# NethermindEth/stark-rings

Measured on AMD Instinct MI355X. Metric: ring-muls/sec (Goldilocks, deg 2^16, batch 2^14), higher is better.
Workload: dtype u64; 1 GPU; goldilocks_d65536_b16384; ring=goldilocks, degree=65536, batch_per_gpu=16384, global_batch=16384, layout=ark-ff Montgomery u64 limbs, in place (a *= b), b read-only, variant=mul, parallelism=batch-sharded x1, twiddle broadcast only

## Files before the change

stark_rings_amd/csrc/ntt_goldilocks.hpp:

```cpp
#pragma once
#include <utility>

#include "fields.hpp"

namespace sr {
namespace gl {

using G = Goldilocks;
typedef uint64_t u64;
typedef uint32_t u32;

constexpr int kW16Exp = 156;

__device__ __forceinline__ u64 ld_stream(const u64 *p) { return __builtin_nontemporal_load(p); }
__device__ __forceinline__ void st_stream(u64 *p, u64 v) { __builtin_nontemporal_store(v, p); }
__device__ __forceinline__ u64 ld_scratch(const u64 *p) { return *p; }
__device__ __forceinline__ void st_scratch(u64 *p, u64 v) { *p = v; }
__device__ __forceinline__ void st_result(u64 *p, u64 v) {
    repcheck::leaves_library(v);
    st_stream(p, v);
}
__device__ __forceinline__ void st_slots(u64 *p, u64 v) {
    repcheck::leaves_library(v);
    *p = v;
// ... 247 lines not shown
template <int E>
SR_HD u64 mul_pow2_signed(u64 x) {
    if constexpr (E == 0) return x;
    else if constexpr (E < 96) return mul_pow2<E>(x);
    else if constexpr (E == 96) return G::neg(x);
    else return G::neg(mul_pow2<E - 96>(x));
}
constexpr int twist_exp(int q) { return (39 << (q + 1)) % 192; }
template <int Q, bool INVERSE, int... Js>
SR_HD void twist_rows(u64 *x, std::integer_sequence<int, Js...>) {
    ((x[Js] = mul_pow2_signed<INVERSE ? (192 - (twist_exp(Q) * (Js & ((16 >> Q) - 1))) % 192) % 192
                                      : (twist_exp(Q) * (Js & ((16 >> Q) - 1))) % 192>(x[Js])),
     ...);
}

struct Tables {
    const u64 *tw, *itw;
    const u64 *twist_f;
    const u64 *twist_i_plain, *twist_i_mul;
    const u64 *w1f, *w1i, *w1i_mul;
    const u64 *w2f, *w2i;
    const u64 *wcf, *wci;
};

template <int M, int DIR, bool TWIST>
__global__ __launch_bounds__(256) void strided_kernel(u64 *data, const u64 *src, int k, int s_lo, const u64 *tw, const u64 *twist) {
    constexpr int R = 1 << M;
    const int ls = k - s_lo - M;
    const size_t S = (size_t)1 << ls;
    const unsigned chunks = (unsigned)(S >> 8);
    const unsigned ci = blockIdx.x % chunks;
    const unsigned rest = blockIdx.x / chunks;
    const unsigned h = rest & ((1u << s_lo) - 1u);
    const size_t poly = rest >> s_lo;
    const unsigned i = ci * 256u + threadIdx.x;
    const size_t off = (poly << k) + ((size_t)h << (k - s_lo)) + i;
    u64 *base = data + off;
    const u64 *sbase = src + off;

    u64 x[R];
#pragma unroll
    for (int j = 0; j < R; j++) x[j] = sbase[(size_t)j << ls];

    if (DIR == 0) {
#pragma unroll
        for (int t = 0; t < M; t++) {
            const int half = 1 << (M - 1 - t);
#pragma unroll
            for (int j = 0; j < R; j++) {
                if (j & half) continue;
                const u64 w = tw[(1u << (s_lo + t)) + (h << t) + (unsigned)(j >> (M - t))];
                const u64 u = x[j], v = G::mul(x[j + half], w);
                x[j] = G::add(u, v);
                x[j + half] = G::sub(u, v);
            }
        }
        if (TWIST) {
#pragma unroll
            for (int j = 0; j < R; j++) x[j] = G::mul(x[j], twist[((size_t)((h << M) + j) << 12) + i]);
        }
    } else {
        if (TWIST) {
#pragma unroll
            for (int j = 0; j < R; j++) x[j] = G::mul(x[j], twist[((size_t)((h << M) + j) << 12) + i]);
        }
#pragma unroll
        for (int t = M - 1; t >= 0; t--) {
            const int half = 1 << (M - 1 - t);
#pragma unroll
            for (int j = 0; j < R; j++) {
                if (j & half) continue;
                const u64 w = tw[(1u << (s_lo + t)) + (h << t) + (unsigned)(j >> (M - t))];
                const u64 u = x[j], v = x[j + half];
                x[j] = G::add(u, v);
                x[j + half] = G::mul(G::sub(u, v), w);
            }
        }
    }
#pragma unroll
    for (int j = 0; j < R; j++) base[(size_t)j << ls] = x[j];
}

__device__ __forceinline__ int pad(int pos);

template <int DIR, bool TWIST>
__global__ __launch_bounds__(256, 4) void strided256_kernel(u64 *data, const u64 *src, int k, int s_lo, const u64 *tw, const u64 *twist) {
    __shared__ u64 lds[kLdsElems];
    const int t = threadIdx.x;
    const int ls = k - s_lo - 8;
    const unsigned chunks = 1u << (ls - 4);
    const unsigned ci = blockIdx.x & (chunks - 1u);
    const unsigned rest = blockIdx.x >> (ls - 4);
    const unsigned h = rest & ((1u << s_lo) - 1u);
    const size_t poly = rest >> s_lo;
    const int col = t & 15, rg = t >> 4;
    const unsigned i = ci * 16u + (unsigned)col;
    const size_t off = (poly << k) + ((size_t)h << (k - s_lo)) + i;
    u64 *base = data + off;
    const u64 *sbase = src + off;
    const int base2 = rg * 256 + col;
    u64 x[16];

    if (DIR == 0) {
#pragma unroll
        for (int jj = 0; jj < 16; jj++) x[jj] = sbase[(size_t)(rg + 16 * jj) << ls];
#pragma unroll
        for (int u = 0; u < 4; u++) {
            const int half = 8 >> u;
#pragma unroll
            for (int jj = 0; jj < 16; jj++) {
                if (jj & half) continue;
                const u64 w = tw[(1u << (s_lo + u)) + (h << u) + (unsigned)(jj >> (4 - u))];
                const u64 a = x[jj], v = G::mul(x[jj + half], w);
                x[jj] = G::add(a, v);
                x[jj + half] = G::sub(a, v);
            }
        }
#pragma unroll
        for (int jj = 0; jj < 16; jj++) lds[pad(jj * 256 + t)] = x[jj];
        __syncthreads();
#pragma unroll
        for (int jj = 0; jj < 16; jj++) x[jj] = lds[pad(base2 + jj * 16)];
#pragma unroll
        for (int u = 0; u < 4; u++) {
            const int half = 8 >> u;
#pragma unroll
            for (int jj = 0; jj < 16; jj++) {
                if (jj & half) continue;
                const u64 w = tw[(1u << (s_lo + 4 + u)) + (h << (4 + u)) + ((unsigned)rg << u) + (unsigned)(jj >> (4 - u))];
                const u64 a = x[jj], v = G::mul(x[jj + half], w);
                x[jj] = G::add(a, v);
                x[jj + half] = G::sub(a, v);
            }
        }
#pragma unroll
        for (int jj = 0; jj < 16; jj++) {
            u64 v = x[jj];
            if (TWIST) v = G::mul(v, twist[((size_t)((h << 8) + (unsigned)(16 * rg + jj)) << 12) + i]);
            base[(size_t)(16 * rg + jj) << ls] = v;
        }
    } else {
#pragma unroll
        for (int jj = 0; jj < 16; jj++) {
            u64 v = sbase[(size_t)(16 * rg + jj) << ls];
            if (TWIST) v = G::mul(v, twist[((size_t)((h << 8) + (unsigned)(16 * rg + jj)) << 12) + i]);
            x[jj] = v;
        }
#pragma unroll
        for (int u = 3; u >= 0; u--) {
            const int half = 8 >> u;
#pragma unroll
            for (int jj = 0; jj < 16; jj++) {
                if (jj & half) continue;
                const u64 w = tw[(1u << (s_lo + 4 + u)) + (h << (4 + u)) + ((unsigned)rg << u) + (unsigned)(jj >> (4 - u))];
                const u64 a = x[jj], b = x[jj + half];
                x[jj] = G::add(a, b);
                x[jj + half] = G::mul(G::sub(a, b), w);
            }
        }
#pragma unroll
        for (int jj = 0; jj < 16; jj++) lds[pad(base2 + jj * 16)] = x[jj];
        __syncthreads();
#pragma unroll
        for (int jj = 0; jj < 16; jj++) x[jj] = lds[pad(jj * 256 + t)];
#pragma unroll
        for (int u = 3; u >= 0; u--) {
            const int half = 8 >> u;
#pragma unroll
            for (int jj = 0; jj < 16; jj++) {
                if (jj & half) continue;
                const u64 w = tw[(1u << (s_lo + u)) + (h << u) + (unsigned)(jj >> (4 - u))];
                const u64 a = x[jj], b = x[jj + half];
                x[jj] = G::add(a, b);
                x[jj + half] = G::mul(G::sub(a, b), w);
            }
        }
#pragma unroll
        for (int jj = 0; jj < 16; jj++) base[(size_t)(rg + 16 * jj) << ls] = x[jj];
    }
}

__device__ __forceinline__ int pad(int pos) { return pos + (pos >> 4); }

constexpr int brv5(int i) { return ((i & 1) << 4) | ((i & 2) << 2) | (i & 4) | ((i & 8) >> 2) | ((i & 16) >> 4); }
constexpr int cols_tw_exp(int i) { return (39 * brv5(i)) % 192; }
template <int U, bool INV>
struct ColsStageOf {
    template <int I>
    struct Bf {
        static constexpr int half = 8 >> U;
        static constexpr int lo = (I / half) * 2 * half + I % half, hi = lo + half;
        static constexpr int e = cols_tw_exp((1 << U) + (lo >> (4 - U)));
        static constexpr int E = INV ? (192 - e) % 192 : e;
    };
};
template <int U, int P = kPhased>
SR_HD void cols_stage_fwd(u64 *x) {
    stage_in_groups<ColsStageOf<U, false>::template Bf, true, 8, P, true>(x);
}
template <int U, int P = kPhased>
SR_HD void cols_stage_inv(u64 *x) {
    stage_in_groups<ColsStageOf<U, true>::template Bf, false, 8, P>(x);
}

template <int LC>
struct ColsTile {
    static constexpr int C = 1 << LC;
    static constexpr int kLanes = 16 * C;
    static constexpr int kElems = LC == 4 ? kLdsElems : 256 * C;
    static __device__ __forceinline__ int idx(int leg, int col) {
        const int pos = leg * C + col;
        return LC == 4 ? pos + (pos >> 4) : pos;
    }
};
template <int DIR, int LC>
__device__ __forceinline__ void cols256_tile(const unsigned tile, u64 *data, const u64 *src, int k, const u64 *__restrict__ wc,
                                             const u64 *__restrict__ twist, u64 *lds) {
    using CT = ColsTile<LC>;
    constexpr int C = CT::C;
    const int t = threadIdx.x;
    const int ls = k - 8;
    const unsigned ci = tile & ((1u << (ls - LC)) - 1u);
    const size_t poly = tile >> (ls - LC);
    const int col = t & (C - 1), rg = t >> LC;
    const unsigned i = ci * (unsigned)C + (unsigned)col;
    char *pb = reinterpret_cast<char *>(data + (poly << k));
    const char *ps = reinterpret_cast<const char *>(src + (poly << k));
    const char *tb = reinterpret_cast<const char *>(twist);
    const unsigned leg = 8u << ls;
    const unsigned offA = (((unsigned)rg << ls) + i) * 8u;
    const unsigned offB = (((unsigned)rg << (ls + 4)) + i) * 8u;
    u64 x[16];

    if (DIR == 0) {
#pragma unroll
        for (int jj = 0; jj < 16; jj++) x[jj] = ld_stream(reinterpret_cast<const u64 *>(ps + (offA + (unsigned)jj * 16u * leg)));
        cols_stage_fwd<0>(x);
        cols_stage_fwd<1>(x);
        cols_stage_fwd<2>(x);
        cols_stage_fwd<3>(x);
#pragma unroll
        for (int h = 0; h < 16; h++) x[h] = G::mul(x[h], wc[h * 16 + rg]);
#pragma unroll
        for (int h = 0; h < 16; h++) lds[CT::idx(16 * h + rg, col)] = x[h];
        __syncthreads();
        u64 tw[16];
#pragma unroll
        for (int sg = 0; sg < 16; sg++) tw[sg] = *reinterpret_cast<const u64 *>(tb + (offB + (unsigned)sg * leg));
#pragma unroll
        for (int j = 0; j < 16; j++) x[j] = lds[CT::idx(16 * rg + j, col)];
        dft16_fwd_hot(x);
#pragma unroll
        for (int sg = 0; sg < 16; sg++)
            st_scratch(reinterpret_cast<u64 *>(pb + (offB + (unsigned)sg * leg)), G::mul(x[sg], tw[sg]));
    } else {
        u64 tw[16];
#pragma unroll
        for (int sg = 0; sg < 16; sg++) {
            x[sg] = ld_scratch(reinterpret_cast<const u64 *>(ps + (offB + (unsigned)sg * leg)));
            tw[sg] = *reinterpret_cast<const u64 *>(tb + (offB + (unsigned)sg * leg));
        }
#pragma unroll
        for (int sg = 0; sg < 16; sg++) x[sg] = G::mul(x[sg], tw[sg]);
        dft16_inv_hot(x);
#pragma unroll
        for (int j = 0; j < 16; j++) lds[CT::idx(16 * rg + j, col)] = x[j];
        __syncthreads();
#pragma unroll
        for (int h = 0; h < 16; h++) x[h] = lds[CT::idx(16 * h + rg, col)];
#pragma unroll
        for (int h = 0; h < 16; h++) x[h] = G::mul(x[h], wc[h * 16 + rg]);
        cols_stage_inv<3>(x);
        cols_stage_inv<2>(x);
        cols_stage_inv<1>(x);
        cols_stage_inv<0>(x);
#pragma unroll
        for (int jj = 0; jj < 16; jj++) st_result(reinterpret_cast<u64 *>(pb + (offA + (unsigned)jj * 16u * leg)), x[jj]);
    }
}

constexpr int kColsXcdGroup = 4;
template <int DIR, int LC>
__global__ __launch_bounds__(16 << LC, 4) void cols256_kernel(u64 *data, const u64 *src, int k, const u64 *__restrict__ wc,
                                                              const u64 *__restrict__ twist, unsigned grouped) {
    __shared__ u64 lds[ColsTile<LC>::kElems];
    __shared__ u64 wl[256];
    if (threadIdx.x < 256) wl[threadIdx.x] = wc[threadIdx.x];
    __syncthreads();
    cols256_tile<DIR, LC>(xcd_tile(blockIdx.x, kColsXcdGroup, grouped), data, src, k, wl, twist, lds);
}
template <int LC>
__global__ __launch_bounds__(16 << LC, 4) void cols256_pair_kernel(u64 *data_a, const u64 *src_a, u64 *data_b, const u64 *src_b, int k,
                                                                   const u64 *__restrict__ wc, const u64 *__restrict__ twist,
                                                                   unsigned grouped, unsigned tiles) {
    __shared__ u64 lds[ColsTile<LC>::kElems];
    __shared__ u64 wl[256];
    if (threadIdx.x < 256) wl[threadIdx.x] = wc[threadIdx.x];
    __syncthreads();
    const unsigned v = xcd_tile(blockIdx.x, kColsXcdGroup, grouped);
    const bool second = v >= tiles;
    cols256_tile<0, LC>(second ? v - tiles : v, second ? data_b : data_a, second ? src_b : src_a, k, wl, twist, lds);
}

template <int DIR>
__global__ __launch_bounds__(256, 3) void cols256_keep_kernel(u64 *data, const u64 *src, u64 *data2, const u64 *src2, int k,
                                                              const u64 *__restrict__ wc, const u64 *__restrict__ twist, unsigned npoly,
                                                              unsigned groups) {
    using CT = ColsTile<4>;
    __shared__ u64 lds[CT::kElems];
    __shared__ u64 wl[256];
    const int t = threadIdx.x;
    wl[t] = wc[t];
    const int ls = k - 8;
    const unsigned chunks = 1u << (ls - 4);
    const unsigned xcd = blockIdx.x & 7u, slot = blockIdx.x >> 3;
    const unsigned ci = slot & (chunks - 1u), grp = slot >> (ls - 4);
    const int col = t & 15, rg = t >> 4;
    const unsigned i = ci * 16u + (unsigned)col;
    const char *tb = reinterpret_cast<const char *>(twist);
    const unsigned leg = 8u << ls;
    const unsigned offA0 = (((unsigned)rg << ls) + i) * 8u;
    const unsigned offB0 = (((unsigned)rg << (ls + 4)) + i) * 8u;
    u64 x[16], tw[16];
#pragma unroll
    for (int sg = 0; sg < 16; sg++) tw[sg] = *reinterpret_cast<const u64 *>(tb + (offB0 + (unsigned)sg * leg));
    __syncthreads();
    const unsigned total = data2 ? 2u * npoly : npoly;
    for (unsigned it = xcd + 8u * grp; it < total; it += 8u * groups) {
        const bool second = it >= npoly;
        const unsigned poly = second ? it - npoly : it;
        char *pb = reinterpret_cast<char *>((second ? data2 : data) + ((size_t)poly << k));
        const char *ps = reinterpret_cast<const char *>((second ? src2 : src) + ((size_t)poly << k));
        unsigned offA = offA0, offB = offB0;
        asm volatile("" : "+v"(offA), "+v"(offB));
        if (DIR == 0) {
#pragma unroll
            for (int jj = 0; jj < 16; jj++) x[jj] = ld_stream(reinterpret_cast<const u64 *>(ps + (offA + (unsigned)jj * 16u * leg)));
            cols_stage_fwd<0>(x);
            cols_stage_fwd<1>(x);
            cols_stage_fwd<2>(x);
            cols_stage_fwd<3>(x);
#pragma unroll
            for (int h = 0; h < 16; h++) {
                x[h] = G::mul(x[h], wl[h * 16 + rg]);
                if ((h & 3) == 3) __builtin_amdgcn_sched_barrier(0);
            }
#pragma unroll
            for (int h = 0; h < 16; h++) lds[CT::idx(16 * h + rg, col)] = x[h];
            __syncthreads();
#pragma unroll
            for (int j = 0; j < 16; j++) x[j] = lds[CT::idx(16 * rg + j, col)];
            dft16_fwd_hot(x);
#pragma unroll
            for (int sg = 0; sg < 16; sg++) st_scratch(reinterpret_cast<u64 *>(pb + (offB + (unsigned)sg * leg)), G::mul(x[sg], tw[sg]));
        } else {
#pragma unroll
            for (int sg = 0; sg < 16; sg++) x[sg] = ld_scratch(reinterpret_cast<const u64 *>(ps + (offB + (unsigned)sg * leg)));
#pragma unroll
            for (int sg = 0; sg < 16; sg++) {
                x[sg] = G::mul(x[sg], tw[sg]);
                if ((sg & 3) == 3) __builtin_amdgcn_sched_barrier(0);
            }
            dft16_inv_hot(x);
#pragma unroll
            for (int j = 0; j < 16; j++) lds[CT::idx(16 * rg + j, col)] = x[j];
            __syncthreads();
#pragma unroll
            for (int h = 0; h < 16; h++) x[h] = lds[CT::idx(16 * h + rg, col)];
#pragma unroll
            for (int h = 0; h < 16; h++) {
                x[h] = G::mul(x[h], wl[h * 16 + rg]);
                if ((h & 3) == 3) __builtin_amdgcn_sched_barrier(0);
            }
            cols_stage_inv<3>(x);
            cols_stage_inv<2>(x);
            cols_stage_inv<1>(x);
            cols_stage_inv<0>(x);
#pragma unroll
            for (int jj = 0; jj < 16; jj++) st_result(reinterpret_cast<u64 *>(pb + (offA + (unsigned)jj * 16u * leg)), x[jj]);
        }
        __syncthreads();
    }
}

template <int Q, bool TW, int P = kPhased, bool CANON = false>
__device__ __forceinline__ void tile_fwd(const u64 *__restrict__ src, u64 *lds, const int t, const Tables &T, u64 *x,
                                         int nvalid) {
    constexpr bool LZ = !TW && Q == 0;
#pragma unroll
    for (int j = 0; j < 16; j++) {
        const int pos = j * 256 + t;
        x[j] = TW ? ld_stream(src + (pos < nvalid ? pos : nvalid - 1)) : ld_scratch(src + pos);
    }
    if (TW) twist_rows<Q, false>(x, std::make_integer_sequence<int, 16>{});
    if constexpr (LZ) dft16_fwd_dit<P, true>(x);
    else dft16_fwd_q<Q, P>(x);
    if (TW) x[0] = G::mul(x[0], T.w1f[t]);
#pragma unroll
    for (int r = 1; r < 16; r++) x[r] = G::mul(x[r], T.w1f[r * 256 + t]);
#pragma unroll
    for (int r = 0; r < 16; r++) lds[pad(r * 256 + t)] = x[r];
    __syncthreads();
    const int i0 = t & 15, base2 = (t >> 4) * 256 + i0;
#pragma unroll
    for (int j = 0; j < 16; j++) x[j] = lds[pad(base2 + j * 16)];
    if constexpr (LZ) dft16_fwd_dit<P, true>(x);
    else dft16_fwd<P>(x);
#pragma unroll
    for (int s = 1; s < 16; s++) x[s] = G::mul(x[s], T.w2f[s * 16 + i0]);
#pragma unroll
    for (int s = 0; s < 16; s++) lds[pad(base2 + s * 16)] = x[s];
    __syncthreads();
#pragma unroll
    for (int j = 0; j < 16; j++) x[j] = lds[17 * t + j];
    if constexpr (LZ) dft16_fwd_dit<P, !CANON>(x);
    else dft16_fwd<P>(x);
}

template <int Q, bool TW, int P = kPhased>
__device__ __forceinline__ void tile_inv(u64 *x, u64 *lds, const int t, const Tables &T, const u64 *w1i,
                                         u64 *__restrict__ dst, int nvalid) {
    constexpr bool LZ = !TW && Q == 0;
    dft16_inv<P, LZ>(x);
#pragma unroll
    for (int j = 0; j < 16; j++) lds[17 * t + j] = x[j];
    __syncthreads();
    const int i0 = t & 15, base2 = (t >> 4) * 256 + i0;
#pragma unroll
    for (int s = 0; s < 16; s++) x[s] = lds[pad(base2 + s * 16)];
#pragma unroll
    for (int s = 1; s < 16; s++) x[s] = G::mul(x[s], T.w2i[s * 16 + i0]);
    if (LZ) x[0] = G::canon(x[0]);
    dft16_inv<P, LZ>(x);
#pragma unroll
    for (int j = 0; j < 16; j++) lds[pad(base2 + j * 16)] = x[j];
    __syncthreads();
#pragma unroll
    for (int r = 0; r < 16; r++) x[r] = lds[pad(r * 256 + t)];
    if (TW) x[0] = G::mul(x[0], w1i[t]);
#pragma unroll
    for (int r = 1; r < 16; r++) x[r] = G::mul(x[r], w1i[r * 256 + t]);
    if (LZ) x[0] = G::canon(x[0]);
    if constexpr (LZ) dft16_inv<P, true>(x);
    else dft16_inv_q<Q, P>(x);
    if (TW) twist_rows<Q, true>(x, std::make_integer_sequence<int, 16>{});
#pragma unroll
    for (int j = 0; j < 16; j++) {
        const int pos = j * 256 + t;
        if (!TW) st_scratch(dst + pos, x[j]);
        else if (pos < nvalid) st_result(dst + pos, x[j]);
    }
}

template <int MODE, int Q, bool TW, int PH = (MODE >= 2 ? (TW ? -1 : 0) : kPhased)>
__global__ __launch_bounds__(256, TW ? 3 : 4) void rows_kernel(u64 *a, const u64 *b, u64 *out, Tables T, const u64 *w1i,
                                                                   size_t n_total) {
    __shared__ u64 lds[kLdsElems];
    __shared__ u64 wl[512];
    const int t = threadIdx.x;
    wl[t] = T.w2f[t];
    wl[256 + t] = T.w2i[t];
    __syncthreads();
    T.w2f = wl;
    T.w2i = wl + 256;
    const size_t base = (size_t)blockIdx.x * kTile;
    int nvalid = kTile;
    if (TW) nvalid = n_total - base < (size_t)kTile ? (int)(n_total - base) : kTile;
    constexpr int P = PH;
    u64 A[16];
    if (MODE == 1) {
#pragma unroll
        for (int j = 0; j < 16; j++) {
            const int pos = j * 256 + t;
            lds[pad(pos)] = a[base + ((!TW || pos < nvalid) ? pos : nvalid - 1)];
        }
        __syncthreads();
#pragma unroll
        for (int j = 0; j < 16; j++) A[j] = lds[17 * t + j];
    } else {
        tile_fwd<Q, TW, P, MODE == 0>(a + base, lds, t, T, A, nvalid);
        if (MODE == 0) {
#pragma unroll
            for (int j = 0; j < 16; j++) lds[17 * t + j] = A[j];
            __syncthreads();
#pragma unroll
            for (int j = 0; j < 16; j++) {
                const int pos = j * 256 + t;
                if (!TW || pos < nvalid) st_slots(a + base + pos, lds[pad(pos)]);
            }
            return;
        }
        u64 B[16];
        __syncthreads();
        if (MODE == 3) {
#pragma unroll
            for (int j = 0; j < 16; j++) {
                const int pos = j * 256 + t;
                lds[pad(pos)] = b[base + ((!TW || pos < nvalid) ? pos : nvalid - 1)];
            }
            __syncthreads();
#pragma unroll
            for (int j = 0; j < 16; j++) B[j] = lds[17 * t + j];
        } else {
            tile_fwd<Q, TW, P>(b + base, lds, t, T, B, nvalid);
        }
#pragma unroll
        for (int j = 0; j < 16; j++) A[j] = G::mul(A[j], B[j]);
    }
    tile_inv<Q, TW, P>(A, lds, t, T, w1i, out + base, nvalid);
}

__device__ __forceinline__ void tile256_load(const u64 *__restrict__ src, const int t, u64 *x) {
    const int i0 = t & 15, base2 = (t >> 4) * 256 + i0;
#pragma unroll
    for (int j = 0; j < 16; j++) x[j] = ld_scratch(src + base2 + j * 16);
}
constexpr int kWaveWords = 1024 + 64;
struct Wave256 {
    unsigned *strided, *own, *coalesced;
    int gpos;
    __device__ __forceinline__ Wave256(unsigned *xw, const int t) {
        const int l = t & 63;
        unsigned *reg = xw + (t >> 6) * kWaveWords;
        strided = reg + 272 * (l >> 4) + (l & 15);
        own = reg + 17 * l;
        coalesced = reg + l + (l >> 4);
        gpos = (t & ~63) * 16 + l;
    }
};
__device__ __forceinline__ void wave_lds_fence() {
    __builtin_amdgcn_fence(__ATOMIC_RELEASE, "wavefront");
    __builtin_amdgcn_wave_barrier();
    __builtin_amdgcn_fence(__ATOMIC_ACQUIRE, "wavefront");
}
template <int WS, int RS>
__device__ __forceinline__ void wave256_exchange(unsigned *wr, const unsigned *rd, u64 *x) {
    unsigned lo[16], hi[16];
#pragma unroll
    for (int s = 0; s < 16; s++) wr[WS * s] = (unsigned)x[s];
    wave_lds_fence();
#pragma unroll
    for (int j = 0; j < 16; j++) lo[j] = rd[RS * j];
    wave_lds_fence();
#pragma unroll
    for (int s = 0; s < 16; s++) wr[WS * s] = (unsigned)(x[s] >> 32);
    wave_lds_fence();
#pragma unroll
    for (int j = 0; j < 16; j++) hi[j] = rd[RS * j];
    wave_lds_fence();
#pragma unroll
    for (int j = 0; j < 16; j++) x[j] = ((u64)hi[j] << 32) | lo[j];
}
template <bool CANON = false>
__device__ __forceinline__ void tile256_fwd_regs(const Wave256 &W, const int t, const Tables &T, u64 *x) {
    const int i0 = t & 15;
    dft16_fwd_hot(x);
#pragma unroll
    for (int s = 1; s < 16; s++) x[s] = G::mul(x[s], T.w2f[s * 16 + i0]);
    wave256_exchange<17, 1>(W.strided, W.own, x);
    dft16_fwd_hot<CANON>(x);
}
template <bool CANON = false>
__device__ __forceinline__ void tile256_fwd(const u64 *__restrict__ src, const Wave256 &W, const int t, const Tables &T, u64 *x) {
    tile256_load(src, t, x);
    tile256_fwd_regs<CANON>(W, t, T, x);
}
__device__ __forceinline__ void tile256_inv(u64 *x, const Wave256 &W, const int t, const Tables &T, u64 *__restrict__ dst) {
    const int i0 = t & 15, base2 = (t >> 4) * 256 + i0;
    dft16_inv_hot(x);
    wave256_exchange<1, 17>(W.own, W.strided, x);
#pragma unroll
    for (int s = 1; s < 16; s++) x[s] = G::mul(x[s], T.w2i[s * 16 + i0]);
    x[0] = G::canon(x[0]);
    dft16_inv_hot(x);
#pragma unroll
    for (int j = 0; j < 16; j++) st_scratch(dst + base2 + j * 16, x[j]);
}
template <int MODE>
__device__ __forceinline__ void rows256_tile(const unsigned tile, u64 *a, const u64 *b, u64 *out, const Tables &T, unsigned *xw) {
    const int t = threadIdx.x;
    const size_t base = (size_t)tile * kTile;
    const Wave256 W(xw, t);
    u64 A[16];
    if (MODE == 1) {
#pragma unroll
        for (int j = 0; j < 16; j++) A[j] = a[base + W.gpos + j * 64];
        wave256_exchange<68, 1>(W.coalesced, W.own, A);
    } else {
        tile256_fwd<MODE == 0>(a + base, W, t, T, A);
        if (MODE == 0) {
            wave256_exchange<1, 68>(W.own, W.coalesced, A);
#pragma unroll
            for (int j = 0; j < 16; j++) st_slots(a + base + W.gpos + j * 64, A[j]);
            return;
        }
        u64 B[16];
        if (MODE == 3) {
#pragma unroll
            for (int j = 0; j < 16; j++) B[j] = b[base + W.gpos + j * 64];
            wave256_exchange<68, 1>(W.coalesced, W.own, B);
        } else {
            tile256_fwd(b + base, W, t, T, B);
        }
#pragma unroll
        for (int j = 0; j < 16; j++) A[j] = G::mul(A[j], B[j]);
    }
    tile256_inv(A, W, t, T, out + base);
}
template <int MODE>
__global__ __launch_bounds__(256, 5) void rows256_kernel(u64 *a, const u64 *b, u64 *out, Tables T) {
    __shared__ unsigned xw[4 * kWaveWords];
    __shared__ u64 wl[512];
    wl[threadIdx.x] = T.w2f[threadIdx.x];
    wl[256 + threadIdx.x] = T.w2i[threadIdx.x];
    __syncthreads();
    T.w2f = wl;
    T.w2i = wl + 256;
    rows256_tile<MODE>(blockIdx.x, a, b, out, T, xw);
}


__device__ __forceinline__ u64 pow_from_bits(const u64 *pw, unsigned e, int k) {
    u64 acc = 1;
    for (int j = 0; j <= k; j++)
        if ((e >> j) & 1u) acc = G::mul(acc, pw[j]);
    return acc;
}
__global__ void build_tables_kernel(int k, int c, const u64 *pows, const u64 *ipows, u64 dinv, u64 dinv_mul, u64 *twist_f,
                                    u64 *twist_i_plain, u64 *twist_i_mul, u64 *w1f, u64 *w1i, u64 *w1i_mul, u64 *w2f,
                                    u64 *w2i, u64 *wcf, u64 *wci) {
    const int q = 12 - (k - c);
    const size_t d = (size_t)1 << k;
    const size_t n = d > 4096 ? d : 4096;
    const unsigned mask2d = (unsigned)(2 * d - 1);
    for (size_t idx = blockIdx.x * (size_t)blockDim.x + threadIdx.x; idx < n; idx += (size_t)gridDim.x * blockDim.x) {
        if (idx < d) {
            unsigned b = (unsigned)(idx >> (k - c)), i = (unsigned)(idx & ((d >> c) - 1));
            unsigned e = (unsigned)(((unsigned long long)(2 * bitrev(b, c) + 1) * i) & mask2d);
            twist_f[idx] = pow_from_bits(pows, e, k);
            u64 inv = pow_from_bits(ipows, e, k);
            twist_i_plain[idx] = G::mul(inv, dinv);
            twist_i_mul[idx] = G::mul(inv, dinv_mul);
        }
        if (idx < 4096) {
            unsigned r = (unsigned)(idx >> 8), i0 = (unsigned)(idx & 255);
            unsigned m0 = bitrev(r & ((1u << (4 - q)) - 1u), 4 - q);
            unsigned e1 = (unsigned)((((unsigned long long)i0 * m0) << (c + 1)) & mask2d);
            if (k <= 12) e1 = (e1 + i0) & mask2d;
            w1f[idx] = pow_from_bits(pows, e1, k);
            const u64 inv1 = pow_from_bits(ipows, e1, k);
            w1i[idx] = k <= 12 ? G::mul(inv1, dinv) : inv1;
            w1i_mul[idx] = k <= 12 ? G::mul(inv1, dinv_mul) : inv1;
        }
        if (idx < 256) {
            unsigned s = (unsigned)(idx >> 4), i0 = (unsigned)(idx & 15);
            unsigned e2 = (unsigned)((((unsigned long long)i0 * bitrev(s, 4)) << (k - 7)) & mask2d);
            w2f[idx] = pow_from_bits(pows, e2, k);
            w2i[idx] = pow_from_bits(ipows, e2, k);
            unsigned e3 = (unsigned)((((unsigned long long)(2 * bitrev(s, 4) + 1) * i0) << (k - 8)) & mask2d);
            wcf[idx] = pow_from_bits(pows, e3, k);
            wci[idx] = pow_from_bits(ipows, e3, k);
        }
    }
}

}

struct GoldilocksFastTables {
    int k = -1;
    int c = 0;
    bool cols256 = false;
    bool keep_cols = true;
    bool split_rows = false;
    bool ready = false;
    gl::Tables t{};
    size_t chunk_polys = 0;
    void (*prof_begin)(void *user, int tag, hipStream_t st) = nullptr;
    void (*prof_end)(void *user, hipStream_t st) = nullptr;
    void *prof_user = nullptr;
};
struct GlProfScope {
    const GoldilocksFastTables &f;
    hipStream_t st;
    GlProfScope(const GoldilocksFastTables &ff, int tag, hipStream_t s) : f(ff), st(s) {
        if (f.prof_begin) f.prof_begin(f.prof_user, tag, st);
    }
    ~GlProfScope() {
        if (f.prof_end) f.prof_end(f.prof_user, st);
    }
};

inline bool gl_fast_supported(const GoldilocksFastTables &f) { return f.ready; }
inline size_t gl_fast_extra_bytes(int k) {
    if (k < 8 || k > 22) return 0;
    return (((size_t)3 << k) + 3 * 4096 + 4 * 256) * sizeof(uint64_t);
}
inline int gl_fast_init(GoldilocksFastTables &f, int k, const uint64_t *tw, const uint64_t *itw, uint64_t *extra,
                        const uint64_t *host_pows, const uint64_t *host_ipows, uint64_t dinv, uint64_t dinv_mul,
                        bool allow_cols256, size_t chunk_polys, hipStream_t st) {
    f.k = k;
    f.ready = false;
    if (gl_fast_extra_bytes(k) == 0) return 0;
    const size_t d = (size_t)1 << k;
    uint64_t *p = extra;
    uint64_t *twist_f = p;            p += d;
    uint64_t *twist_ip = p;           p += d;
    uint64_t *twist_im = p;           p += d;
    uint64_t *w1f = p;                p += 4096;
    uint64_t *w1i = p;                p += 4096;
    uint64_t *w1im = p;               p += 4096;
    uint64_t *w2f = p;                p += 256;
    uint64_t *w2i = p;                p += 256;
    uint64_t *wcf = p;                p += 256;
    uint64_t *wci = p;
    f.cols256 = k >= 16 && k <= 20 && allow_cols256;
    f.chunk_polys = chunk_polys;
    f.c = f.cols256 ? 8 : (k > 12 ? k - 12 : 0);
    uint64_t *d_pows = nullptr;
    if (hipMalloc(&d_pows, 2 * (k + 1) * sizeof(uint64_t)) != hipSuccess) return 1;
    bool ok = hipMemcpy(d_pows, host_pows, (k + 1) * 8, hipMemcpyHostToDevice) == hipSuccess &&
              hipMemcpy(d_pows + k + 1, host_ipows, (k + 1) * 8, hipMemcpyHostToDevice) == hipSuccess;
    if (ok) {
        unsigned blocks = (unsigned)(((d > 4096 ? d : 4096) + 255) / 256);
        if (blocks > 4096) blocks = 4096;
        hipLaunchKernelGGL(gl::build_tables_kernel, dim3(blocks), dim3(256), 0, st, k, f.c, d_pows, d_pows + k + 1, dinv, dinv_mul,
                           twist_f, twist_ip, twist_im, w1f, w1i, w1im, w2f, w2i, wcf, wci);
        ok = hipGetLastError() == hipSuccess;
        ok = hipStreamSynchronize(st) == hipSuccess && ok;
    }
    (void)hipFree(d_pows);
    if (!ok) return 1;
    f.t = gl::Tables{tw, itw, twist_f, twist_ip, twist_im, w1f, w1i, w1im, w2f, w2i, wcf, wci};
    f.ready = true;
    return 0;
}
inline void gl_fast_destroy(GoldilocksFastTables &f) { f.ready = false; }

template <int DIR, bool TWIST>
inline int gl_launch_strided(const GoldilocksFastTables &f, int M, uint64_t *data, const uint64_t *src, int k, int s_lo,
                             size_t npoly, const uint64_t *tw, const uint64_t *twist, hipStream_t st) {
    GlProfScope ps(f, DIR == 0 ? 0 : 2, st);
    const size_t S = (size_t)1 << (k - s_lo - M);
    const size_t blocks = npoly * ((size_t)1 << s_lo) * (S >> 8);
    if (blocks == 0 || blocks > 0x7FFFFFFFull) return 1;
    dim3 g((unsigned)blocks), b(256);
    switch (M) {
        case 0: hipLaunchKernelGGL((gl::strided_kernel<0, DIR, TWIST>), g, b, 0, st, data, src, k, s_lo, tw, twist); break;
        case 1: hipLaunchKernelGGL((gl::strided_kernel<1, DIR, TWIST>), g, b, 0, st, data, src, k, s_lo, tw, twist); break;
        case 2: hipLaunchKernelGGL((gl::strided_kernel<2, DIR, TWIST>), g, b, 0, st, data, src, k, s_lo, tw, twist); break;
        case 3: hipLaunchKernelGGL((gl::strided_kernel<3, DIR, TWIST>), g, b, 0, st, data, src, k, s_lo, tw, twist); break;
        case 4: hipLaunchKernelGGL((gl::strided_kernel<4, DIR, TWIST>), g, b, 0, st, data, src, k, s_lo, tw, twist); break;
        default: return 1;
    }
    return hipGetLastError() != hipSuccess;
}
template <int DIR, bool TWIST>
inline int gl_launch_strided256(const GoldilocksFastTables &f, uint64_t *data, const uint64_t *src, int k, int s_lo, size_t npoly,
                                const uint64_t *tw, const uint64_t *twist, hipStream_t st) {
    GlProfScope ps(f, DIR == 0 ? 0 : 2, st);
    const size_t S = (size_t)1 << (k - s_lo - 8);
    const size_t blocks = npoly * ((size_t)1 << s_lo) * (S >> 4);
    if (blocks == 0 || blocks > 0x7FFFFFFFull) return 1;
    hipLaunchKernelGGL((gl::strided256_kernel<DIR, TWIST>), dim3((unsigned)blocks), dim3(256), 0, st, data, src, k, s_lo, tw,
                       twist);
    return hipGetLastError() != hipSuccess;
}
inline int gl_plan(int c, int *ms) {
    int n = 0;
    const bool big = c >= 8;
    if (big) c -= 8;
    while (c > 0) {
        int m = c > 4 ? (c + 1) / 2 : c;
        ms[n++] = m;
        c -= m;
    }
    if (big) ms[n++] = 8;
    return n;
}
template <int DIR>
inline int gl_launch_cols256(const GoldilocksFastTables &f, uint64_t *data, const uint64_t *src, size_t npoly,
                             const uint64_t *wc, const uint64_t *twist, hipStream_t st) {
    GlProfScope ps(f, DIR == 0 ? 0 : 2, st);
    constexpr int LC = 4;
    const size_t blocks = npoly << (f.k - 8 - LC);
    if (blocks == 0 || blocks > 0x7FFFFFFFull) return 1;
    const unsigned grouped = xcd_grouped_tiles(blocks, gl::kColsXcdGroup);
    hipLaunchKernelGGL((gl::cols256_kernel<DIR, LC>), dim3((unsigned)blocks), dim3(16 << LC), 0, st, data, src, f.k, wc, twist,
                       grouped);
    return hipGetLastError() != hipSuccess;
}
template <int DIR>
inline int gl_launch_cols256_lane(const GoldilocksFastTables &f, uint64_t *data, const uint64_t *src, size_t npoly, const uint64_t *wc,
                                  const uint64_t *twist, hipStream_t st) {
    const unsigned chunks = 1u << (f.k - 12);
    unsigned groups = chunks >= 128 ? 1u : 128u / chunks;
    if (!f.keep_cols || f.k != 16 || (npoly & 7u) != 0 || npoly < 16u || npoly > 0x7FFFFFFFull)
        return gl_launch_cols256<DIR>(f, data, src, npoly, wc, twist, st);
    if (groups > npoly / 16) groups = (unsigned)(npoly / 16);
    GlProfScope ps(f, DIR == 0 ? 0 : 2, st);
    hipLaunchKernelGGL((gl::cols256_keep_kernel<DIR>), dim3(8u * chunks * groups), dim3(256), 0, st, data, src, (uint64_t *)nullptr,
                       (const uint64_t *)nullptr, f.k, wc, twist, (unsigned)npoly, groups);
    return hipGetLastError() != hipSuccess;
}
inline int gl_launch_cols256_pair_plain(const GoldilocksFastTables &f, uint64_t *da, const uint64_t *sa, uint64_t *db, const uint64_t *sb,
                                        size_t npoly, hipStream_t st) {
    GlProfScope ps(f, 0, st);
    constexpr int LC = 4;
    const size_t blocks = npoly << (f.k - 8 - LC);
    if (blocks == 0 || blocks > 0x3FFFFFFFull) return 1;
    hipLaunchKernelGGL((gl::cols256_pair_kernel<LC>), dim3((unsigned)(2 * blocks)), dim3(16 << LC), 0, st, da, sa, db, sb, f.k, f.t.wcf,
                       f.t.twist_f, xcd_grouped_tiles(2 * blocks, gl::kColsXcdGroup), (unsigned)blocks);
    return hipGetLastError() != hipSuccess;
}
inline int gl_launch_cols256_lane_pair(const GoldilocksFastTables &f, uint64_t *da, const uint64_t *sa, uint64_t *db, const uint64_t *sb,
                                       size_t npoly, hipStream_t st) {
    const unsigned chunks = 1u << (f.k - 12);
    unsigned groups = chunks >= 128 ? 1u : 128u / chunks;
    if (!f.keep_cols || f.k != 16 || (npoly & 7u) != 0 || npoly < 16u || npoly > 0x3FFFFFFFull)
        return gl_launch_cols256_pair_plain(f, da, sa, db, sb, npoly, st);
    if (groups > npoly / 16) groups = (unsigned)(npoly / 16);
    GlProfScope ps(f, 0, st);
    hipLaunchKernelGGL((gl::cols256_keep_kernel<0>), dim3(8u * chunks * groups), dim3(256), 0, st, da, sa, db, sb, f.k, f.t.wcf, f.t.twist_f,
                       (unsigned)npoly, groups);
    return hipGetLastError() != hipSuccess;
}
inline int gl_strided_fwd(const GoldilocksFastTables &f, uint64_t *d, const uint64_t *src, size_t npoly, hipStream_t st) {
    if (f.cols256) return gl_launch_cols256<0>(f, d, src, npoly, f.t.wcf, f.t.twist_f, st);
    int ms[8];
    const int n = gl_plan(f.k > 12 ? f.k - 12 : 0, ms);
    int s_lo = 0;
    for (int p = 0; p < n; p++) {
        const bool last = p == n - 1;
        const uint64_t *from = p == 0 ? src : d;
        int rc;
        if (ms[p] == 8)
            rc = last ? gl_launch_strided256<0, true>(f, d, from, f.k, s_lo, npoly, f.t.tw, f.t.twist_f, st)
                      : gl_launch_strided256<0, false>(f, d, from, f.k, s_lo, npoly, f.t.tw, nullptr, st);
        else
            rc = last ? gl_launch_strided<0, true>(f, ms[p], d, from, f.k, s_lo, npoly, f.t.tw, f.t.twist_f, st)
                      : gl_launch_strided<0, false>(f, ms[p], d, from, f.k, s_lo, npoly, f.t.tw, nullptr, st);
        if (rc) return rc;
        s_lo += ms[p];
    }
    return 0;
}
inline int gl_strided_inv(const GoldilocksFastTables &f, uint64_t *d, size_t npoly, bool fused, hipStream_t st) {
    const uint64_t *tw_i = fused ? f.t.twist_i_mul : f.t.twist_i_plain;
    if (f.cols256) return gl_launch_cols256<1>(f, d, d, npoly, f.t.wci, tw_i, st);
    int ms[8];
    const int n = gl_plan(f.k > 12 ? f.k - 12 : 0, ms);
    int s_lo = f.k > 12 ? f.k - 12 : 0;
    for (int p = n - 1; p >= 0; p--) {
        s_lo -= ms[p];
        const bool first = p == n - 1;
        int rc;
        if (ms[p] == 8)
            rc = first ? gl_launch_strided256<1, true>(f, d, d, f.k, s_lo, npoly, f.t.itw, tw_i, st)
                       : gl_launch_strided256<1, false>(f, d, d, f.k, s_lo, npoly, f.t.itw, nullptr, st);
        else
            rc = first ? gl_launch_strided<1, true>(f, ms[p], d, d, f.k, s_lo, npoly, f.t.itw, tw_i, st)
                       : gl_launch_strided<1, false>(f, ms[p], d, d, f.k, s_lo, npoly, f.t.itw, nullptr, st);
        if (rc) return rc;
    }
    return 0;
}
template <int MODE>
inline int gl_launch_rows(const GoldilocksFastTables &f, uint64_t *a, const uint64_t *b, uint64_t *out, size_t npoly,
                          bool fused, hipStream_t st) {
    const size_t n_total = npoly << f.k;
    const size_t tiles = (n_total + gl::kTile - 1) / gl::kTile;
    if (tiles == 0 || tiles > 0x7FFFFFFFull) return 1;
    GlProfScope ps(f, 1, st);
    const uint64_t *w1i = fused ? f.t.w1i_mul : f.t.w1i;
    dim3 g((unsigned)tiles), blk(256);
#define SR_GL_ROWS(QQ, TT) hipLaunchKernelGGL((gl::rows_kernel<MODE, QQ, TT>), g, blk, 0, st, a, b, out, f.t, w1i, n_total)
    const bool tw = f.c == 0;
    switch (f.k - f.c) {
        case 8:
            if (tw) SR_GL_ROWS(4, true);
            else hipLaunchKernelGGL((gl::rows256_kernel<MODE>), g, blk, 0, st, a, b, out, f.t);
            break;
        case 9: if (tw) SR_GL_ROWS(3, true); else SR_GL_ROWS(3, false); break;
        case 10: if (tw) SR_GL_ROWS(2, true); else SR_GL_ROWS(2, false); break;
        case 11: if (tw) SR_GL_ROWS(1, true); else SR_GL_ROWS(1, false); break;
        default: if (tw) SR_GL_ROWS(0, true); else SR_GL_ROWS(0, false); break;
    }
#undef SR_GL_ROWS
    return hipGetLastError() != hipSuccess;
}
inline int gl_fast_fwd(const GoldilocksFastTables &f, uint64_t *d, size_t batch, hipStream_t st) {
    if (batch == 0) return 0;
    if (gl_strided_fwd(f, d, d, batch, st)) return 1;
    return gl_launch_rows<0>(f, d, nullptr, d, batch, false, st);
}
inline int gl_fast_inv(const GoldilocksFastTables &f, uint64_t *d, size_t batch, hipStream_t st) {
    if (batch == 0) return 0;
    if (gl_launch_rows<1>(f, d, nullptr, d, batch, false, st)) return 1;
    return gl_strided_inv(f, d, batch, false, st);
}
inline int gl_fast_ring_mul(const GoldilocksFastTables &f, uint64_t *out, const uint64_t *a, const uint64_t *b, uint64_t *scratch,
                            size_t scratch_polys, size_t batch, hipStream_t st) {
    if (batch == 0) return 0;
    if (f.k <= 12)
        return gl_launch_rows<2>(f, const_cast<uint64_t *>(a), b, out, batch, true, st);
    if (scratch_polys == 0) return 1;
    size_t chunk = f.chunk_polys ? f.chunk_polys : batch;
    if (chunk > scratch_polys) chunk = scratch_polys;
    const size_t stride = (size_t)1 << f.k;
    for (size_t e = 0; e < batch; e += chunk) {
        const size_t n = batch - e < chunk ? batch - e : chunk;
        uint64_t *o = out + e * stride;
        if (f.cols256) {
            if (gl_launch_cols256_pair_plain(f, o, a + e * stride, scratch, b + e * stride, n, st)) return 1;
        } else {
            if (gl_strided_fwd(f, o, a + e * stride, n, st)) return 1;
            if (gl_strided_fwd(f, scratch, b + e * stride, n, st)) return 1;
        }
        if (f.split_rows) {
            if (gl_launch_rows<0>(f, scratch, nullptr, scratch, n, false, st)) return 1;
            if (gl_launch_rows<3>(f, o, scratch, o, n, true, st)) return 1;
        } else if (gl_launch_rows<2>(f, o, scratch, o, n, true, st)) {
// ... 69 lines not shown
```

Baseline: 1.103 million ring-muls/s.

## Specialize keep kernel to degree 2^16 and overlap table loads with data loads

The column keep kernel now hard-codes k=16 and builds addresses from a scalar base plus a fixed leg stride in the global address space, so per-element address arithmetic becomes cheaper. Loading the twiddle and column tables is moved inside the first loop iteration, after the data loads are issued, so table latency overlaps with them. The barrier at the end of each iteration is replaced by a barrier before the LDS write, and LDS indexing switches to precomputed padded pointers. The rows kernel likewise issues its tile loads before staging the twiddle tables into LDS. This hard-codes the degree (the k argument is ignored) and reorders barriers, which adds correctness risk.

```diff
diff --git a/stark_rings_amd/csrc/ntt_goldilocks.hpp b/stark_rings_amd/csrc/ntt_goldilocks.hpp
--- a/stark_rings_amd/csrc/ntt_goldilocks.hpp
+++ b/stark_rings_amd/csrc/ntt_goldilocks.hpp
@@ -573,30 +573,42 @@
     cols256_tile<0, LC>(second ? v - tiles : v, second ? data_b : data_a, second ? src_b : src_a, k, wl, twist, lds);
 }
 
+constexpr long kKeepLeg = 2048;
+typedef __attribute__((address_space(1))) char *keep_gptr;
+typedef __attribute__((address_space(1))) u64 *keep_gword;
+__device__ __forceinline__ keep_gptr keep_scalar(const char *base) {
+    u64 b = reinterpret_cast<u64>(base);
+    asm("" : "+s"(b));
+    return (keep_gptr)b;
+}
+__device__ __forceinline__ keep_gword keep_ptr_a(const char *base, unsigned off, int jj) {
+    return (keep_gword)(keep_scalar(base + jj * 16 * kKeepLeg) + off);
+}
+__device__ __forceinline__ keep_gword keep_ptr_b(const char *base, unsigned off, int sg) {
+    return (keep_gword)((keep_scalar(base + ((sg >> 2) * 4 + 2) * kKeepLeg) + off) + ((sg & 3) - 2) * kKeepLeg);
+}
 template <int DIR>
-__global__ __launch_bounds__(256, 3) void cols256_keep_kernel(u64 *data, const u64 *src, u64 *data2, const u64 *src2, int k,
+__global__ __launch_bounds__(256, 3) void cols256_keep_kernel(u64 *data, const u64 *src, u64 *data2, const u64 *src2, int ,
                                                               const u64 *__restrict__ wc, const u64 *__restrict__ twist, unsigned npoly,
                                                               unsigned groups) {
     using CT = ColsTile<4>;
+    constexpr int k = 16, ls = 8;
     __shared__ u64 lds[CT::kElems];
     __shared__ u64 wl[256];
     const int t = threadIdx.x;
-    wl[t] = wc[t];
-    const int ls = k - 8;
-    const unsigned chunks = 1u << (ls - 4);
     const unsigned xcd = blockIdx.x & 7u, slot = blockIdx.x >> 3;
-    const unsigned ci = slot & (chunks - 1u), grp = slot >> (ls - 4);
+    const unsigned ci = slot & 15u, grp = slot >> 4;
     const int col = t & 15, rg = t >> 4;
     const unsigned i = ci * 16u + (unsigned)col;
     const char *tb = reinterpret_cast<const char *>(twist);
-    const unsigned leg = 8u << ls;
     const unsigned offA0 = (((unsigned)rg << ls) + i) * 8u;
     const unsigned offB0 = (((unsigned)rg << (ls + 4)) + i) * 8u;
-    u64 x[16], tw[16];
-#pragma unroll
-    for (int sg = 0; sg < 16; sg++) tw[sg] = *reinterpret_cast<const u64 *>(tb + (offB0 + (unsigned)sg * leg));
-    __syncthreads();
+    u64 *const lh = lds + 17 * rg + col;
+    u64 *const lj = lds + 272 * rg + col;
+    static_assert(CT::kElems == 17 * 256, "padded tile: 17 words per leg");
+    u64 x[16], tw[16], wv = 0;
     const unsigned total = data2 ? 2u * npoly : npoly;
+    bool first = true;
     for (unsigned it = xcd + 8u * grp; it < total; it += 8u * groups) {
         const bool second = it >= npoly;
         const unsigned poly = second ? it - npoly : it;
@@ -606,38 +618,55 @@
         asm volatile("" : "+v"(offA), "+v"(offB));
         if (DIR == 0) {
 #pragma unroll
-            for (int jj = 0; jj < 16; jj++) x[jj] = ld_stream(reinterpret_cast<const u64 *>(ps + (offA + (unsigned)jj * 16u * leg)));
+            for (int jj = 0; jj < 16; jj++) x[jj] = __builtin_nontemporal_load(keep_ptr_a(ps, offA, jj));
+            if (first) {
+                wv = wc[t];
+    #pragma unroll
+            for (int sg = 0; sg < 16; sg++) tw[sg] = *keep_ptr_b(tb, offB, sg);
+            }
             cols_stage_fwd<0>(x);
             cols_stage_fwd<1>(x);
             cols_stage_fwd<2>(x);
             cols_stage_fwd<3>(x);
+            if (first) {
+                wl[t] = wv;
+                __syncthreads();
+            }
 #pragma unroll
             for (int h = 0; h < 16; h++) {
                 x[h] = G::mul(x[h], wl[h * 16 + rg]);
                 if ((h & 3) == 3) __builtin_amdgcn_sched_barrier(0);
             }
-#pragma unroll
-            for (int h = 0; h < 16; h++) lds[CT::idx(16 * h + rg, col)] = x[h];
+            if (!first) __syncthreads();
+#pragma unroll
+            for (int h = 0; h < 16; h++) lh[272 * h] = x[h];
             __syncthreads();
 #pragma unroll
-            for (int j = 0; j < 16; j++) x[j] = lds[CT::idx(16 * rg + j, col)];
+            for (int j = 0; j < 16; j++) x[j] = lj[17 * j];
             dft16_fwd_hot(x);
 #pragma unroll
-            for (int sg = 0; sg < 16; sg++) st_scratch(reinterpret_cast<u64 *>(pb + (offB + (unsigned)sg * leg)), G::mul(x[sg], tw[sg]));
+            for (int sg = 0; sg < 16; sg++) *keep_ptr_b(pb, offB, sg) = G::mul(x[sg], tw[sg]);
         } else {
 #pragma unroll
-            for (int sg = 0; sg < 16; sg++) x[sg] = ld_scratch(reinterpret_cast<const u64 *>(ps + (offB + (unsigned)sg * leg)));
+            for (int sg = 0; sg < 16; sg++) x[sg] = *keep_ptr_b(ps, offB, sg);
+            if (first) {
+                wv = wc[t];
+    #pragma unroll
+            for (int sg = 0; sg < 16; sg++) tw[sg] = *keep_ptr_b(tb, offB, sg);
+            }
 #pragma unroll
             for (int sg = 0; sg < 16; sg++) {
                 x[sg] = G::mul(x[sg], tw[sg]);
                 if ((sg & 3) == 3) __builtin_amdgcn_sched_barrier(0);
             }
             dft16_inv_hot(x);
-#pragma unroll
-            for (int j = 0; j < 16; j++) lds[CT::idx(16 * rg + j, col)] = x[j];
+            if (first) wl[t] = wv;
+            else __syncthreads();
+#pragma unroll
+            for (int j = 0; j < 16; j++) lj[17 * j] = x[j];
             __syncthreads();
 #pragma unroll
-            for (int h = 0; h < 16; h++) x[h] = lds[CT::idx(16 * h + rg, col)];
+            for (int h = 0; h < 16; h++) x[h] = lh[272 * h];
 #pragma unroll
             for (int h = 0; h < 16; h++) {
                 x[h] = G::mul(x[h], wl[h * 16 + rg]);
@@ -648,9 +677,12 @@
             cols_stage_inv<1>(x);
             cols_stage_inv<0>(x);
 #pragma unroll
-            for (int jj = 0; jj < 16; jj++) st_result(reinterpret_cast<u64 *>(pb + (offA + (unsigned)jj * 16u * leg)), x[jj]);
-        }
-        __syncthreads();
+            for (int jj = 0; jj < 16; jj++) {
+                repcheck::leaves_library(x[jj]);
+                __builtin_nontemporal_store(x[jj], keep_ptr_a(pb, offA, jj));
+            }
+        }
+        first = false;
     }
 }
 
@@ -848,7 +880,7 @@
     for (int j = 0; j < 16; j++) st_scratch(dst + base2 + j * 16, x[j]);
 }
 template <int MODE>
-__device__ __forceinline__ void rows256_tile(const unsigned tile, u64 *a, const u64 *b, u64 *out, const Tables &T, unsigned *xw) {
+__device__ __forceinline__ void rows256_tile(const unsigned tile, u64 *a, const u64 *b, u64 *out, Tables T, unsigned *xw, u64 *wl) {
     const int t = threadIdx.x;
     const size_t base = (size_t)tile * kTile;
     const Wave256 W(xw, t);
@@ -856,9 +888,18 @@
     if (MODE == 1) {
 #pragma unroll
         for (int j = 0; j < 16; j++) A[j] = a[base + W.gpos + j * 64];
+    } else {
+        tile256_load(a + base, t, A);
+    }
+    wl[t] = T.w2f[t];
+    wl[256 + t] = T.w2i[t];
+    __syncthreads();
+    T.w2f = wl;
+    T.w2i = wl + 256;
+    if (MODE == 1) {
         wave256_exchange<68, 1>(W.coalesced, W.own, A);
     } else {
-        tile256_fwd<MODE == 0>(a + base, W, t, T, A);
+        tile256_fwd_regs<MODE == 0>(W, t, T, A);
         if (MODE == 0) {
             wave256_exchange<1, 68>(W.own, W.coalesced, A);
 #pragma unroll
@@ -882,12 +923,7 @@
 __global__ __launch_bounds__(256, 5) void rows256_kernel(u64 *a, const u64 *b, u64 *out, Tables T) {
     __shared__ unsigned xw[4 * kWaveWords];
     __shared__ u64 wl[512];
-    wl[threadIdx.x] = T.w2f[threadIdx.x];
-    wl[256 + threadIdx.x] = T.w2i[threadIdx.x];
-    __syncthreads();
-    T.w2f = wl;
-    T.w2i = wl + 256;
-    rows256_tile<MODE>(blockIdx.x, a, b, out, T, xw);
+    rows256_tile<MODE>(blockIdx.x, a, b, out, T, xw, wl);
 }
 
 
```

New measurement: 1.120 million ring-muls/s (median of 6 runs). 1.02x the previous value.
